# nobodyscool/vkComputeShader_tinyraytracer

Hardware: AMD Instinct MI355X
Metric: Mray/s (primary+secondary) at 1024×768 depth4; 1/2/4/8-GPU scaling (higher is better)
Workload: dtype f32; 1 GPU; C2: 1024x768, 4 spheres + floor + 7616x3808 seeded envmap, depth 4, 1 spp; width=1024, height=768, max_depth=4, spp=1, parallelism=1 GPU

## Files before the change

vkcomputeshader_tinyraytracer_amd/csrc/sky_spans.cpp:

```cpp
#include "sky_spans.h"

#include <algorithm>
#include <cmath>
#include <initializer_list>

#include "../../include/trt/abi.h"
#include "trt_bands.h"

namespace trt {
namespace {

struct Range {
    double lo = 1e300, hi = -1e300;
    void add(double v) {
        lo = std::min(lo, v);
        hi = std::max(hi, v);
    }
};

struct Ball {
    double qx, qy, qz, R, K, dz;
    double ex[2], ey[2];
    double ylo, yhi;
    double a, inv_a;
// ... 21 lines not shown
            const double disc = b * b - a * c;
            if (disc < 0.0) continue;
            const double s = std::sqrt(disc);
            r.add((-b + s) * inv_a);
            r.add((-b - s) * inv_a);
        }
    }
};

struct Seg2 {
    double x0, y0, x1, y1;
    double inv_dy;
};

struct Group {
    bool full = false;
    int nball = 0, nseg = 0;
    Ball ball[4];
    Seg2 seg[12];
};

constexpr double kHuge = 1e6;

bool finite3(const float* v) { return std::isfinite(v[0]) && std::isfinite(v[1]) && std::isfinite(v[2]); }

void prepare_group(const SpanIn& in, const float* cams, uint32_t n, Group& G) {
    const double dz = (double)in.dz;
    double lo[3] = {1e300, 1e300, 1e300}, hi[3] = {-1e300, -1e300, -1e300};
    for (uint32_t f = 0; f < n; ++f) {
        if (!finite3(cams + 3 * f)) {
            G.full = true;
            return;
        }
        for (int a = 0; a < 3; ++a) {
            lo[a] = std::min(lo[a], (double)cams[3 * f + a]);
            hi[a] = std::max(hi[a], (double)cams[3 * f + a]);
        }
    }
    const double oc[3] = {0.5 * (lo[0] + hi[0]), 0.5 * (lo[1] + hi[1]), 0.5 * (lo[2] + hi[2])};
    double rho = 0.0;
    for (uint32_t f = 0; f < n; ++f) {
        double d2 = 0.0;
        for (int a = 0; a < 3; ++a) d2 += ((double)cams[3 * f + a] - oc[a]) * ((double)cams[3 * f + a] - oc[a]);
        rho = std::max(rho, std::sqrt(d2));
    }
    if (!(rho < kHuge) || !(std::fabs(oc[0]) < kHuge) || !(std::fabs(oc[1]) < kHuge) || !(std::fabs(oc[2]) < kHuge)) {
// ... 62 lines not shown
            if (sg.y1 != sg.y0) sg.inv_dy = 1.0 / (sg.y1 - sg.y0);
            G.seg[G.nseg++] = sg;
        }
    }
}

void seg_extent(const Seg2& s, double dy_lo, double dy_hi, Range& r) {
    if (std::max(s.y0, s.y1) < dy_lo || std::min(s.y0, s.y1) > dy_hi) return;
    double t0 = 0.0, t1 = 1.0;
    if (s.inv_dy != 0.0) {
        double ta = (dy_lo - s.y0) * s.inv_dy, tb = (dy_hi - s.y0) * s.inv_dy;
        if (ta > tb) std::swap(ta, tb);
        t0 = std::max(t0, ta);
        t1 = std::min(t1, tb);
        if (t0 > t1) return;
    }
    r.add(s.x0 + t0 * (s.x1 - s.x0));
    r.add(s.x0 + t1 * (s.x1 - s.x0));
}

}

uint32_t sky_spans(const SpanIn& in, const float* cams, uint32_t nframes, uint32_t group_frames, uint32_t* out,
                   uint32_t* ntr_out, uint32_t* shift_out) {
    *ntr_out = 0;
    *shift_out = 0;
    const bool banded = in.band_rows != 0 && in.band_count > 1;
    if (in.rays_in || nframes == 0 || in.width == 0 || in.height == 0) return 0;
    if (banded && (in.band_rows % 8u != 0 || in.band_index >= in.band_count)) return 0;
    const uint32_t rows = banded ? band_group_rows(in.height, in.band_rows, in.band_count, in.band_index) : in.height;
    const uint32_t ntr = (rows + 7u) / 8u, ntx = (in.width + 7u) / 8u;
    if (ntr == 0 || ntr > kSpanWords) return 0;
    uint32_t shift = 1;
    while ((1u << shift) < group_frames && shift < 16) ++shift;
    if (group_frames == 0) shift = 16;
    auto tables = [&](uint32_t s) { return (nframes + (1u << s) - 1u) >> s; };
    while (tables(shift) > kSpanMaxTables || tables(shift) * ntr > kSpanWords) ++shift;
    const uint32_t T = tables(shift);
    *ntr_out = ntr;
    *shift_out = shift;

    const bool sane = in.dz < 0.0f && in.dz > -1e9f;
    const double W = (double)in.width, H = (double)in.height;
    for (uint32_t g = 0; g < T; ++g) {
        uint32_t* tab = out + (size_t)g * ntr;
        const uint32_t f0 = g << shift, n = std::min(nframes - f0, 1u << shift);
        Group G;
        if (sane) prepare_group(in, cams + 3 * (size_t)f0, n, G);
        else G.full = true;
        for (uint32_t tr = 0; tr < ntr; ++tr) {
            if (G.full) {
                tab[tr] = kSpanFull;
                continue;
            }
            const uint32_t k0 = tr * 8u, k1 = std::min(k0 + 7u, rows - 1u);
            const uint32_t y0 = banded ? band_frame_row(k0, in.band_rows, in.band_count, in.band_index) : k0;
            const uint32_t y1 = y0 + (k1 - k0);
            const double dy_hi = H * 0.5 - (double)y0 + 8.0;
            const double dy_lo = H * 0.5 - (double)(y1 + 1u) - ((in.flags & TRT_FLAG_ROW_QUIRK) ? 1.0 : 0.0) - 8.0;
            Range r;
            for (int i = 0; i < G.nball; ++i) G.ball[i].extent(dy_lo, dy_hi, r);
            for (int i = 0; i < G.nseg; ++i) seg_extent(G.seg[i], dy_lo, dy_hi, r);
            if (!(r.lo <= r.hi)) {
                tab[tr] = (r.lo == 1e300 && r.hi == -1e300) ? 0u : kSpanFull;
                continue;
            }
            const double x0 = std::floor(r.lo + W * 0.5 - 0.5), x1 = std::ceil(r.hi + W * 0.5 - 0.5);
            const double c0 = std::max(0.0, std::floor(x0 / 8.0) - 1.0);
            const double c1 = std::min((double)ntx, std::floor(x1 / 8.0) + 2.0);
            tab[tr] = c0 < c1 ? ((uint32_t)c0 | ((uint32_t)c1 << 16)) : 0u;
        }
    }
    return T;
}

}

extern "C" int trt_diag_sky_spans(uint32_t width, uint32_t height, float fov, uint32_t flags, uint32_t band_rows,
                                  uint32_t band_count, uint32_t band_index, int rays_in, const float* spheres,
                                  const float* cams, uint32_t nframes, uint32_t group_frames, uint32_t* out,
                                  uint32_t out_cap, uint32_t* ntr, uint32_t* shift) {
    if (!spheres || !cams || !out || !ntr || !shift) return -1;
    trt::SpanIn in{};
    in.width = width;
    in.height = height;
    in.dz = (float)(-1.0 * ((double)height / (2.0 * std::tan((double)fov / 2.0))));
    in.flags = flags;
    in.band_rows = band_rows;
    in.band_count = band_count;
    in.band_index = band_index;
    in.rays_in = rays_in != 0;
    for (int i = 0; i < 4; ++i)
        for (int a = 0; a < 4; ++a) in.sph[i][a] = spheres[4 * i + a];
    uint32_t tmp[trt::kSpanWords];
    const uint32_t T = trt::sky_spans(in, cams, nframes, group_frames, tmp, ntr, shift);
    if ((size_t)T * *ntr > out_cap) return -1;
    std::copy(tmp, tmp + (size_t)T * *ntr, out);
    return (int)T;
}
```

vkcomputeshader_tinyraytracer_amd/csrc/sky_spans.h:

```cpp
#pragma once

#include <stdint.h>

namespace trt {

constexpr uint32_t kSpanWords = 384;
constexpr uint32_t kSpanMaxTables = 4;
constexpr uint32_t kSpanFull = 0xffff0000u;

struct SpanIn {
    uint32_t width, height;
    float dz;
    uint32_t flags;
    uint32_t band_rows, band_count, band_index;
    bool rays_in;
    float sph[4][4];
};

uint32_t sky_spans(const SpanIn& in, const float* cams, uint32_t nframes, uint32_t group_frames, uint32_t* out,
                   uint32_t* ntr, uint32_t* shift);

}
```

vkcomputeshader_tinyraytracer_amd/csrc/trt_ctx.h:

```cpp
#pragma once

#include <hip/hip_runtime.h>

#include <string>
#include <vector>

#include "../../include/trt/abi.h"
#include "shadow_mask.h"
#include "trt_device.h"

#ifndef TRT_BUILD_MAX_IN_FLIGHT
#define TRT_BUILD_MAX_IN_FLIGHT TRT_MAX_FRAMES_IN_FLIGHT
#endif
static_assert(TRT_BUILD_MAX_IN_FLIGHT >= 1u && TRT_BUILD_MAX_IN_FLIGHT <= TRT_MAX_FRAMES_IN_FLIGHT,
              "TRT_BUILD_MAX_IN_FLIGHT must lie in [1, TRT_MAX_FRAMES_IN_FLIGHT]");

struct trt_ctx {
    int device = 0;
    hipStream_t own_stream = nullptr;
    hipStream_t stream = nullptr;
    std::string err;
    trt_ubo ubo{};
    bool have_scene = false;

    trt::BatchRec* d_batches = nullptr;
    float4* d_nodes = nullptr;
    trt::BvhNode* d_bvh = nullptr;
    trt::Bvh4Node* d_bvh4 = nullptr;
    trt::Bvh4QNode* d_bvh4q = nullptr;
    trt::TriGeo* d_bvh_tris = nullptr;
    uint32_t node_off[11] = {0};
    uint32_t top = 0;
    trt::TriGeo* d_geo = nullptr;
    trt::TriShade* d_shade = nullptr;
    trt::Mat* d_mats = nullptr;
    uint32_t* d_env = nullptr;
    uint2* d_envp = nullptr;
    size_t envp_cap = 0;
    bool envp_ok = false;
    uint32_t nbatch = 0, ntri = 0, nmat = 0, env_w = 0, env_h = 0;
    uint32_t* d_sky = nullptr;
    size_t sky_cap = 0;
    bool sky_on = true, sky_ok = false;
    bool span_on = true;
    uint32_t span_frames = 16;
    uint16_t* d_smask = nullptr;
    bool smask_on = true, smask_ok = false;
    float smask_cell = trt::kShadowCellDefault;
    trt::ShadowMaskIn smask_key{};
    uint32_t smask_nx = 1, smask_nz = 1, smask_rows[2] = {0x0FFF0FFFu, 0x0FFF0FFFu};
    float smask_inv = 0.0f;
    bool smask_fallback = true;
    uint64_t env_gen = 0;
    struct SkyKey {
        uint32_t width, height, flags;
        float dz;
        uint64_t env_gen;
    } sky_key{};

    void* d_out8 = nullptr;
    size_t cap8 = 0;
    void* d_out32 = nullptr;
    size_t cap32 = 0;
    void* d_rays = nullptr;
    size_t caprays = 0;
    unsigned long long* d_counters = nullptr;
    uint32_t num_cus = 256;
    hipEvent_t ev0 = nullptr, ev1 = nullptr;
// ... 80 lines not shown
```

vkcomputeshader_tinyraytracer_amd/csrc/trt_device.h:

```cpp
#pragma once

#include <stdint.h>

#include <hip/hip_runtime.h>

#include "sky_spans.h"

namespace trt {

struct alignas(32) BatchRec {
    float bmin[3];
    float bmax[3];
    int32_t start;
    int32_t count_ni;
};
static_assert(sizeof(BatchRec) == 32, "BatchRec is one s_load_dwordx8");

struct alignas(16) TriGeo {
    float v0[3];
    float e1[3];
    float e2[3];
    float pad[3];
};
static_assert(sizeof(TriGeo) == 48, "TriGeo is 3 x dwordx4");
// ... 151 lines not shown
    float4* __restrict__ diag;
    uint32_t defer;
    uint32_t ev_cap;
    uint32_t shq_cap;
    float4* __restrict__ ev;
    float4* __restrict__ shq;
    uint2* __restrict__ px_ev;
    uint32_t* __restrict__ fb;
    DeferCtr* __restrict__ dctr;
    uint32_t defer_sub;
    uint32_t dframes;
    uint32_t defer_inter;
    uint32_t px_fstride;
    size_t ev_fstride, shq_fstride;
    uint32_t spp_lanes;
    FrameRec fr[kMaxLaunchFrames];
    const uint32_t* __restrict__ sky;
    uint32_t span_tables, span_shift, span_ntr;
    uint32_t span[kSpanWords];
    const uint16_t* __restrict__ smask;
    uint32_t smask_nx, smask_nz;
    float smask_inv;
    uint32_t smask_rows[2];
};
static_assert(sizeof(KArgs) <= 4096, "KArgs fits the 4 KB kernel-argument limit");

}
```

vkcomputeshader_tinyraytracer_amd/csrc/trt_kernel.hip:

```cpp
#include <hip/hip_runtime.h>

#include <algorithm>


#include "../../include/trt/abi.h"
#include "trt_bands.h"
#include "trt_device.h"
#include "trt_math.h"

namespace trt {

__device__ __forceinline__ void wave_lds_sync() { __syncthreads(); }
__device__ __forceinline__ uint32_t lane_id() { return threadIdx.x; }
__device__ __forceinline__ uint32_t lane_rank(uint64_t mask) {
    return __builtin_amdgcn_mbcnt_hi((uint32_t)(mask >> 32), __builtin_amdgcn_mbcnt_lo((uint32_t)mask, 0u));
}

#define TRT_EPS 0.0001f
#ifndef TRT_SKIP_DARK
#define TRT_SKIP_DARK 1
#endif
#ifndef TRT_SPEC_SKIP
#define TRT_SPEC_SKIP 1
#endif
// ... 1878 lines not shown
    }
    if (F.out8) F.out8[o] = pack_rgba8(A, g);
}

__device__ __forceinline__ uint32_t span_word(const KArgs& A, uint32_t tile, uint32_t f) {
    if (A.span_tables == 0u || tile >= A.ntiles) return kSpanFull;
    return A.span[(f >> A.span_shift) * A.span_ntr + tile / A.ntx];
}
__device__ __forceinline__ bool span_outside(const KArgs& A, uint32_t tile, uint32_t span) {
    const uint32_t col = tile % A.ntx;
    return col < (span & 0xffffu) || col >= (span >> 16);
}

__device__ __forceinline__ void sky_tile_store(const KArgs& A, uint32_t tile, const FrameRec& F0, const FrameRec* F1) {
    const uint32_t lane = lane_id();
    const uint32_t x = (tile % A.ntx) * 8u + (lane & 7u), k = (tile / A.ntx) * 8u + (lane >> 3);
    if (x >= A.width || k >= A.rows) return;
    const uint32_t word = A.sky[(size_t)band_row(A, k) * A.width + x];
    const size_t o = (size_t)k * A.width + x;
    if (F0.out8) F0.out8[out_index(A, F0, o)] = word;
    if (F1 && F1->out8) F1->out8[out_index(A, *F1, o)] = word;
}

template <int CAP, bool COUNT, int GEOM, bool SPLIT, bool DEFER = false, bool HYB = SPLIT, bool SKY = false,
          bool SMASK = false>
__device__ __forceinline__ void trace_tile(const KArgs& A, const FrameRec& F, uint32_t tile, Cnt& cnt, float* lds,
                                           float4* slab, uint32_t sub = 0, uint32_t frame = 0) {
    const uint32_t lane = lane_id();
    if (tile >= A.ntiles) return;
    const uint32_t x = (tile % A.ntx) * 8u + (lane & 7u);
    uint32_t k = (tile / A.ntx) * 8u + (lane >> 3);
    const f3 orig = mk(F.cam[0], F.cam[1], F.cam[2]);
    if constexpr (DEFER) {
        const uint32_t S = (!SPLIT && A.defer_sub > 1u) ? A.defer_sub : 1u, rows = 8u / S;
        k = (tile / A.ntx) * 8u + sub * rows + (lane >> 3);
        const bool valid = x < A.width && k < A.rows && (lane >> 3) < rows;
        EvLog L;
        L.S = dscratch(A, frame);
        L.stripe = ((tile * S + sub) * 0x9E3779B1u) >> (32 - 7);
        static_assert(kDeferStripes == 128u, "stripe hash yields 7 bits");
        const size_t o = valid ? (size_t)k * A.width + x : 0u;
        const Seg root = valid ? Seg{orig, primary_dir(A, x, band_row(A, k), 0), 1.0f, 0} : Seg{orig, orig, 0.0f, 0};
        defer_walk<GEOM, SPLIT>(A, lds, slab, L, valid, root, kEvRoot, (uint32_t)o);
        return;
    }
    if (x >= A.width || k >= A.rows) return;
// ... 156 lines not shown
}

template <int GEOM>
constexpr int slab_float4s() {
    return GEOM == 1 ? 64 * 3 : GEOM >= 2 ? (bvh_lds_entries<GEOM>() > 0 ? bvh_lds_entries<GEOM>() * 16 : 1) : 1;
}
#ifndef TRT_G0_WAVES
#define TRT_G0_WAVES 5
#endif
template <int GEOM, int CAP = 99>
constexpr int waves_per_simd() {
    return GEOM == 3 ? (CAP <= 3 ? TRT_G3_WAVES_SHALLOW : TRT_G3_WAVES) : GEOM == 0 ? TRT_G0_WAVES : TRT_WAVES;
}

#ifndef TRT_DEFER_WAVES
#define TRT_DEFER_WAVES 4
#endif
template <int GEOM, int CAP, bool SPLIT, bool DEFER>
constexpr int trace_waves() {
    return (DEFER && GEOM == 3) ? TRT_DEFER_WAVES : waves_per_simd<GEOM, ((SPLIT || DEFER) ? 99 : CAP)>();
}

template <int CAP, bool COUNT, int GEOM, bool SPLIT, bool DEFER, bool HYB, bool SKY, bool SPANS = false,
          bool SMASK = false>
__device__ __forceinline__ void trace_body(const KArgs& A) {
    static_assert(!SPANS || SKY, "the sky spans cull into the sky table");
    static_assert(!SMASK || SPANS, "the occluder masks ride on the span kernel");
    __shared__ float lds[DEFER ? defer_pool_floats() : lds_stack_floats<CAP, GEOM, HYB>()];
    __shared__ float4 slab[slab_float4s<GEOM>()];
    const uint32_t vb = blockIdx.x;
    Cnt cnt;
#ifdef TRT_DIAG_WAVE_CLOCK
    const uint64_t t_start = __builtin_amdgcn_s_memrealtime();
#endif
    uint32_t f = 0, t = vb, tile;
    if (!SPLIT && !DEFER && A.spp_lanes) {
        const uint32_t per = A.ntiles * A.spp;
        f = vb / per;
        const uint32_t r = vb - f * per;
        trace_samples<CAP, COUNT, GEOM>(A, A.fr[f], xcd_tile(A, r / A.spp), r % A.spp, cnt, lds, slab);
        if (COUNT) flush_counts(A, cnt);
        return;
    }
    if (!SPLIT && !DEFER && A.nframes > 1u) {
        if (A.xcd_inter && A.frame_group > 1u && (GEOM == 0 || TRT_MESH_PAIRS)) {
            uint32_t pr;
            tile = inter_tile(A, vb, pr, (A.nframes + 1u) / 2u);
            f = 2u * pr;
#ifndef TRT_DIAG_TRIVIAL
            if constexpr (SPANS) {
                if (span_outside(A, tile, span_word(A, tile, f))) {
                    sky_tile_store(A, tile, A.fr[f], f + 1u < A.nframes ? &A.fr[f + 1u] : nullptr);
                    return;
                }
            }
#endif
            trace_tile<CAP, COUNT, GEOM, SPLIT, DEFER, HYB, SKY, SMASK>(A, A.fr[f], tile, cnt, lds, slab);
            if (f + 1u < A.nframes) trace_tile<CAP, COUNT, GEOM, SPLIT, DEFER, HYB, SKY, SMASK>(A, A.fr[f + 1u], tile, cnt, lds, slab);
            if (COUNT) flush_counts(A, cnt);
            return;
        } else if (A.xcd_inter) {
            tile = inter_tile(A, vb, f, A.nframes);
        } else {
            f = vb / A.ntiles;
            t = vb - f * A.ntiles;
            tile = xcd_tile(A, t, f);
        }
    } else if (DEFER && !SPLIT) {
        const uint32_t Sd = A.defer_sub > 1u ? A.defer_sub : 1u, per = A.ntiles * Sd;
        if (A.defer_inter && A.dframes > 1u) {
            const uint32_t F = A.dframes, per8 = per & ~7u;
            if (vb < F * per8) {
                const uint32_t x = vb & 7u, j = vb >> 3;
// ... 7 lines not shown
        } else {
            f = vb / per;
            t = vb - f * per;
        }
        tile = xcd_tile(A, t / Sd);
        trace_tile<CAP, COUNT, GEOM, SPLIT, DEFER, HYB>(A, A.fr[f], tile, cnt, lds, slab, t % Sd, f);
#ifdef TRT_DIAG_WAVE_CLOCK
        if (threadIdx.x == 0 && A.out32 && A.dframes <= 1u) {
            const uint64_t t_end = __builtin_amdgcn_s_memrealtime();
            uint32_t* rec = reinterpret_cast<uint32_t*>(A.out32) + 4 * (size_t)blockIdx.x;
            uint32_t xcc;
            asm volatile("s_getreg_b32 %0, hwreg(HW_REG_XCC_ID)" : "=s"(xcc));
            rec[0] = tile | ((xcc & 15u) << 28);
            rec[1] = (uint32_t)t_start;
            rec[2] = (uint32_t)(t_end - t_start);
            rec[3] = (uint32_t)(t_start >> 32);
        }
#endif
        return;
    } else {
        tile = xcd_tile(A, t);
    }
#if !defined(TRT_DIAG_TRIVIAL) && !defined(TRT_DIAG_WAVE_CLOCK)
    if constexpr (SPANS) {
        if (span_outside(A, tile, span_word(A, tile, f))) {
            sky_tile_store(A, tile, A.fr[f], nullptr);
            return;
        }
    }
#endif
    trace_tile<CAP, COUNT, GEOM, SPLIT, DEFER, HYB, SKY, SMASK>(A, A.fr[f], tile, cnt, lds, slab);
#ifdef TRT_DIAG_WAVE_CLOCK
    __syncthreads();
    float* clk = A.out32 ? A.out32 : reinterpret_cast<float*>(A.diag);
    if (threadIdx.x == 0 && clk) {
        const uint64_t t_end = __builtin_amdgcn_s_memrealtime();
        uint32_t* rec = reinterpret_cast<uint32_t*>(clk) + 4 * (size_t)blockIdx.x;
        uint32_t xcc;
        asm volatile("s_getreg_b32 %0, hwreg(HW_REG_XCC_ID)" : "=s"(xcc));
        rec[0] = (A.out32 ? xcd_tile(A, blockIdx.x) : (tile | (f << 20))) | ((xcc & 15u) << 28);
        rec[1] = (uint32_t)t_start;
        rec[2] = (uint32_t)(t_end - t_start);
        rec[3] = (uint32_t)(t_start >> 32);
    }
#endif
    if (COUNT) flush_counts(A, cnt);
}

template <int CAP, bool COUNT, int GEOM, bool SPLIT, bool DEFER = false, bool HYB = SPLIT>
__global__ __launch_bounds__(64, (trace_waves<GEOM, CAP, SPLIT, DEFER>())) void trace_kernel(KArgs A) {
    trace_body<CAP, COUNT, GEOM, SPLIT, DEFER, HYB, false>(A);
}

template <int CAP>
__global__ __launch_bounds__(64, (trace_waves<0, CAP, false, false>())) void sky_trace_kernel(KArgs A) {
    trace_body<CAP, false, 0, false, false, false, true, true>(A);
}
template <int CAP>
__global__ __launch_bounds__(64, (trace_waves<0, CAP, false, false>())) void sky_trace_kernel_nospan(KArgs A) {
    trace_body<CAP, false, 0, false, false, false, true, false>(A);
}
template <int CAP>
__global__ __launch_bounds__(64, (trace_waves<0, CAP, false, false>())) void sky_trace_kernel_smask(KArgs A) {
    trace_body<CAP, false, 0, false, false, false, true, true, true>(A);
}

template <int CAP, bool COUNT, int GEOM, bool DEFER = false>
__global__ __launch_bounds__(64, waves_per_simd<GEOM>()) void trace_tasks(KArgs A) {
    __shared__ float lds[DEFER ? defer_pool_floats() : lds_stack_floats<CAP, GEOM, true>()];
    __shared__ float4 slab[slab_float4s<GEOM>()];
    Cnt cnt;
    const uint32_t n = min(*A.q_in_n, A.q_cap);
    for (uint32_t base = blockIdx.x * 64u; base < n; base += gridDim.x * 64u) {
        const uint32_t t = base + threadIdx.x;
        if constexpr (DEFER) {
            const bool valid = t < n;
            Seg root{mk(0.0f, 0.0f, 0.0f), mk(0.0f, 0.0f, 0.0f), 0.0f, 0};
            uint32_t pixel = 0, link = kEvRoot;
            if (valid) {
                const float4* q = reinterpret_cast<const float4*>(A.q_in + t);
                const float4 a = q[0], b = q[1];
                const uint32_t pd = __float_as_uint(b.w);
                pixel = pd >> kTaskDepthBits;
                root = Seg{mk(a.x, a.y, a.z), mk(a.w, b.x, b.y), b.z, (int)(pd & ((1u << kTaskDepthBits) - 1u))};
                link = A.q_link_in[t];
            }
            EvLog L;
// ... 285 lines not shown
        else if (geom == 1) TRT_SPLIT_G(CAP, 1);  \
        else if (geom == 2) TRT_SPLIT_G(CAP, 2);  \
        else TRT_SPLIT_G(CAP, 3);                 \
    } while (0)
        switch (A.split_w) {
        case 2: TRT_SPLIT(1); break;
        case 3: TRT_SPLIT(2); break;
        case 4: TRT_SPLIT(3); break;
        default: TRT_SPLIT(4); break;
        }
#undef TRT_SPLIT
#undef TRT_SPLIT_G
        return hipGetLastError();
    }
    const uint32_t fblocks = A.spp_lanes ? std::max(A.nframes, 1u) * A.spp
                             : A.nframes > 1u && A.xcd_inter && A.frame_group > 1u && (geom == 0 || TRT_MESH_PAIRS)
                                 ? (A.nframes + 1u) / 2u
                                 : std::max(A.nframes, 1u);
    const dim3 fgrid(A.ntiles * fblocks);
    const bool sky = A.sky && geom == 0 && !count && A.spp <= 1 && !A.rays_in && !A.out32;
#define TRT_LAUNCH_G(CAP, G)                                                                             \
    do {                                                                                                 \
        if (count) hipLaunchKernelGGL((trace_kernel<CAP, true, G, false>), fgrid, block, 0, stream, A);  \
        else if (G == 0 && sky && A.span_tables && A.smask) hipLaunchKernelGGL((sky_trace_kernel_smask<CAP>), fgrid, block, 0, stream, A); \
        else if (G == 0 && sky && A.span_tables) hipLaunchKernelGGL((sky_trace_kernel<CAP>), fgrid, block, 0, stream, A); \
        else if (G == 0 && sky) hipLaunchKernelGGL((sky_trace_kernel_nospan<CAP>), fgrid, block, 0, stream, A); \
        else hipLaunchKernelGGL((trace_kernel<CAP, false, G, false>), fgrid, block, 0, stream, A);       \
    } while (0)
#define TRT_LAUNCH(CAP)                          \
    do {                                         \
        if (geom == 0) TRT_LAUNCH_G(CAP, 0);     \
        else if (geom == 1) TRT_LAUNCH_G(CAP, 1); \
        else if (geom == 2) TRT_LAUNCH_G(CAP, 2); \
        else TRT_LAUNCH_G(CAP, 3);               \
    } while (0)
    if (D <= 1) TRT_LAUNCH(0);
    else if (D <= 2) TRT_LAUNCH(1);
    else if (D <= 3) TRT_LAUNCH(2);
    else if (D <= 4) TRT_LAUNCH(3);
    else if (D <= 5) TRT_LAUNCH(4);
    else if (D <= 8) TRT_LAUNCH(7);
    else TRT_LAUNCH(19);
#undef TRT_LAUNCH
#undef TRT_LAUNCH_G
    return hipGetLastError();
}
// ... 83 lines not shown
```

vkcomputeshader_tinyraytracer_amd/csrc/trt_runtime.cpp:

```cpp
#include <hip/hip_runtime.h>

#include <algorithm>
#include <cmath>
#include <cstddef>
#include <cstdio>
#include <cstdlib>
#include <limits>
#include <cstring>
#include <map>
#include <new>
#include <string>
#include <vector>

#include "../../include/trt/abi.h"
#include "jpeg.h"
#include "trt_bands.h"
#include "trt_ctx.h"
#include "trt_device.h"

namespace trt {
hipError_t touch_stream(hipStream_t s, void* scratch) {
    hipError_t e = hipMemsetAsync(scratch, 0, 4, s);
    return e == hipSuccess ? hipStreamSynchronize(s) : e;
}
// ... 179 lines not shown
    }
    if (const char* e = std::getenv("TRT_BVH_WAVES4")) c->bvh_waves4 = std::atoi(e) != 0 ? 1 : 0;
    if (const char* e = std::getenv("TRT_SPP_LANES")) c->spp_lanes = std::atoi(e) != 0;
    if (const char* e = std::getenv("TRT_DEFER_PPW")) {
        const int ppw = std::atoi(e);
        c->defer_sub = ppw == 8 ? 8u : ppw == 16 ? 4u : ppw == 32 ? 2u : ppw == 64 ? 1u : 0u;
    }
    if (const char* e = std::getenv("GPU_MAX_HW_QUEUES")) c->hw_queues = (uint32_t)std::max(1, std::atoi(e));
    if (const char* e = std::getenv("TRT_DEFER_INTER")) c->defer_inter = (uint32_t)std::min(2, std::max(0, std::atoi(e)));
    if (const char* e = std::getenv("TRT_DEFER_GROUP"))
        c->defer_group = (uint32_t)std::min((int)trt::kMaxLaunchFrames, std::max(1, std::atoi(e)));
    if (const char* e = std::getenv("TRT_DEFER_IN_FLIGHT")) {
        c->defer_in_flight = (uint32_t)std::min((int)TRT_BUILD_MAX_IN_FLIGHT, std::max(1, std::atoi(e)));
        c->defer_in_flight_set = true;
    }
    if (const char* e = std::getenv("TRT_XCD_ROT")) c->xcd_rot = (uint32_t)std::min(8, std::max(0, std::atoi(e)));
    if (const char* e = std::getenv("TRT_XCD_SKEW")) c->xcd_skew = (uint32_t)std::min(7, std::max(0, std::atoi(e)));
    if (const char* e = std::getenv("TRT_XCD_INTER")) c->xcd_inter = (uint32_t)std::min(2, std::max(0, std::atoi(e)));
    if (const char* e = std::getenv("TRT_FRAME_GROUP")) c->frame_group = std::min(2, std::max(1, std::atoi(e)));
    if (const char* e = std::getenv("TRT_SKY_TABLE")) c->sky_on = std::atoi(e) != 0;
    if (const char* e = std::getenv("TRT_SKY_SPANS")) c->span_on = std::atoi(e) != 0;
    if (const char* e = std::getenv("TRT_SKY_SPAN_FRAMES")) c->span_frames = (uint32_t)std::min(64, std::max(0, std::atoi(e)));
    if (const char* e = std::getenv("TRT_SHADOW_MASK")) c->smask_on = std::atoi(e) != 0;
    if (const char* e = std::getenv("TRT_SHADOW_MASK_CELL")) {
        const float v = (float)std::atof(e);
        if (v > 0.0f) c->smask_cell = v;
    }
    *out = c;
    return TRT_OK;
}

int trt_destroy(trt_ctx* c) {
    if (!c) return TRT_ERR_INVALID;
    (void)hipSetDevice(c->device);
    if (c->own_stream) (void)hipStreamSynchronize(c->own_stream);
    if (c->stream && c->stream != c->own_stream) (void)hipStreamSynchronize(c->stream);
    (void)hipDeviceSynchronize();
    free_scene(c);
    (void)hipFree(c->d_envp);
    (void)hipFree(c->d_sky);
    (void)hipFree(c->d_smask);
    (void)hipFree(c->d_out8);
    (void)hipFree(c->d_out32);
    (void)hipFree(c->d_rays);
    (void)hipFree(c->d_counters);
    for (hipEvent_t e : c->fev) (void)hipEventDestroy(e);
// ... 321 lines not shown
            (void)hipFree(c->d_sky);
            c->d_sky = nullptr;
            c->sky_cap = 0;
            const hipError_t e = hipMalloc((void**)&c->d_sky, bytes);
            if (e == hipErrorOutOfMemory) {
                (void)hipGetLastError();
                c->d_sky = nullptr;
                c->sky_key = key;
                c->sky_ok = true;
                return TRT_OK;
            }
            HIP_TRY(c, e);
            c->sky_cap = bytes;
        }
        HIP_TRY(c, trt::launch_sky(A, c->d_sky, stream));
        HIP_TRY(c, hipStreamSynchronize(stream));
        c->sky_key = key;
        c->sky_ok = true;
    }
    A.sky = c->d_sky;
    return TRT_OK;
}

void fill_spans(const trt_ctx* c, KArgs& A) {
    A.span_tables = 0;
    if (!A.sky || !c->span_on || A.out32 || A.spp > 1) return;
    trt::SpanIn in{};
    in.width = A.width;
    in.height = A.height;
    in.dz = A.dz;
    in.flags = A.flags;
    in.band_rows = A.band_rows;
    in.band_count = A.band_count;
    in.band_index = A.band_index;
    in.rays_in = A.rays_in != nullptr;
    for (int i = 0; i < 4; ++i) {
        for (int a = 0; a < 3; ++a) in.sph[i][a] = A.sph[i].c[a];
        in.sph[i][3] = A.sph[i].r;
    }
    float cams[3 * trt::kMaxLaunchFrames];
    const uint32_t n = std::min(A.nframes, trt::kMaxLaunchFrames);
    for (uint32_t f = 0; f < n; ++f)
        for (int a = 0; a < 3; ++a) cams[3 * f + a] = A.fr[f].cam[a];
    uint32_t ntr = 0, shift = 0;
    const uint32_t T = trt::sky_spans(in, cams, n, c->span_frames, A.span, &ntr, &shift);
    if (T == 0 || A.ntx == 0 || ntr != A.ntiles / A.ntx) return;
    A.span_tables = T;
    A.span_shift = shift;
    A.span_ntr = ntr;
}

int attach_smask(trt_ctx* c, KArgs& A, hipStream_t stream) {
    A.smask = nullptr;
    if (!A.sky || !A.span_tables || !c->smask_on) return TRT_OK;
    trt::ShadowMaskIn key{};
    for (int j = 0; j < 4; ++j) {
        for (int a = 0; a < 3; ++a) key.sph[j][a] = A.sph[j].c[a];
        key.sph[j][3] = A.sph[j].r;
    }
    std::memcpy(key.light, A.light, sizeof(key.light));
    key.flags = A.flags & TRT_FLAG_SPHERES;
    if (!c->smask_ok || std::memcmp(&key, &c->smask_key, sizeof(key)) != 0) {
        c->smask_ok = false;
        trt::ShadowMask m;
        trt::shadow_mask(key, c->smask_cell, true, m);
        constexpr size_t kCells = 200u * 250u;
        if (m.cells.size() > kCells) trt::shadow_mask(key, c->smask_cell, false, m);
        if (!m.fallback) {
// ... 13 lines not shown
                HIP_TRY(c, hipStreamSynchronize(stream));
            }
        }
        c->smask_nx = m.nx;
        c->smask_nz = m.nz;
        c->smask_inv = m.inv_cell;
        c->smask_rows[0] = m.rows[0] | (m.rows[1] << 16);
        c->smask_rows[1] = m.rows[2] | (m.rows[3] << 16);
        c->smask_fallback = m.fallback;
        c->smask_key = key;
        c->smask_ok = true;
    }
    if (!c->d_smask || c->smask_fallback) return TRT_OK;
    for (uint32_t f = 0; f < A.nframes && f < trt::kMaxLaunchFrames; ++f)
        for (int a = 0; a < 3; ++a)
            if (!(std::fabs(A.fr[f].cam[a]) <= trt::kShadowCamMax)) return TRT_OK;
    A.smask = c->d_smask;
    A.smask_nx = c->smask_nx;
    A.smask_nz = c->smask_nz;
    A.smask_inv = c->smask_inv;
    A.smask_rows[0] = c->smask_rows[0];
    A.smask_rows[1] = c->smask_rows[1];
    return TRT_OK;
}

int check_params(trt_ctx* c, const trt_params* p) {
    if (!p) return fail(c, TRT_ERR_INVALID, "trt_render: null params");
    if (!c->have_scene) return fail(c, TRT_ERR_NOSCENE, "trt_render: no scene uploaded");
    if (p->width == 0 || p->height == 0 || p->width > 65536 || p->height > 65536)
        return fail(c, TRT_ERR_INVALID, "trt_render: image size out of range");
    if (p->max_depth < 1 || p->max_depth > TRT_MAX_DEPTH_LIMIT)
        return fail(c, TRT_ERR_INVALID, "trt_render: max_depth must be 1..20");
    if (p->spp > 4096) return fail(c, TRT_ERR_INVALID, "trt_render: spp must be <= 4096");
    if (p->band_rows && p->band_count > 1 && p->band_index >= p->band_count)
        return fail(c, TRT_ERR_INVALID, "trt_render: band_index >= band_count");
    if ((p->flags & TRT_FLAG_BAND_IN_PLACE) && !(p->flags & TRT_FLAG_DEVICE_PTRS))
        return fail(c, TRT_ERR_INVALID, "trt_render: TRT_FLAG_BAND_IN_PLACE needs TRT_FLAG_DEVICE_PTRS");
    if ((p->flags & TRT_FLAG_ENVMAP) && !c->d_env)
        return fail(c, TRT_ERR_INVALID, "trt_render: TRT_FLAG_ENVMAP without an uploaded envmap");
    return TRT_OK;
}

void fill_args(trt_ctx* c, const trt_params* p, KArgs& A) {
    std::memset(&A, 0, sizeof(A));
    A.width = p->width;
    A.height = p->height;
// ... 342 lines not shown
        HIP_TRY(c, hipStreamCreateWithFlags(&s, hipStreamNonBlocking));
        HIP_TRY(c, trt::touch_stream(s, c->d_counters));
        c->aux.push_back(s);
        hipEvent_t e;
        HIP_TRY(c, hipEventCreateWithFlags(&e, hipEventDisableTiming));
        c->aux_ev.push_back(e);
    }
    if (nfl > 1) {
        if (!c->fork_ev) HIP_TRY(c, hipEventCreateWithFlags(&c->fork_ev, hipEventDisableTiming));
        HIP_TRY(c, hipEventRecord(c->fork_ev, c->stream));
        for (uint32_t k = 0; k + 1 < nfl; ++k) {
            HIP_TRY(c, hipStreamWaitEvent(c->aux[k], c->fork_ev, 0));
            sv.push_back(c->aux[k]);
        }
    }
    for (uint32_t j = 0; j < nl; ++j) {
        const uint32_t i0 = first[j], n = first[j + 1] - i0;
        c->ubo = ubo_of(i0);
        fill_ubo_args(A, c->ubo);
        A.nframes = n;
        for (uint32_t k = 0; k < n; ++k) fill_frame(A.fr[k], ubo_of(i0 + k), frames[i0 + k].out8, frames[i0 + k].in_place);
        fill_spans(c, A);
        if ((rc = attach_smask(c, A, c->stream)) != TRT_OK) return rc;
        uint32_t slot = j % nfl;
        if ((rc = prepare_split(c, p, A, slot, sv[slot])) != TRT_OK) {
            if (c->frames_in_flight || slot == 0 || rc != TRT_ERR_OOM) return rc;
            (void)hipGetLastError();
            c->err.clear();
            nfl = slot;
            c->cur_in_flight = nfl;
            slot = j % nfl;
            if ((rc = prepare_split(c, p, A, slot, sv[slot])) != TRT_OK) return rc;
        }
        hipStream_t st = sv[slot];
        const bool timed = timing && j % every == 0;
        const size_t k = 2 * (size_t)(j / every);
        if (timed) HIP_TRY(c, hipEventRecord(c->fev[k], st));
        HIP_TRY(c, trt::launch_trace(A, st, false));
        if ((rc = fence_split(c, A, slot, st)) != TRT_OK) return rc;
        if (timed) {
            HIP_TRY(c, hipEventRecord(c->fev[k + 1], st));
            c->fev_nframes.push_back(n);
            c->fev_frames = j / every + 1;
        }
    }
    c->ubo = ubo_of(nframes - 1);
// ... 70 lines not shown
            HIP_TRY(c, hipMemcpyAsync(c->d_rays, p->rays_in, bytes, hipMemcpyHostToDevice, c->stream));
            A.rays_in = reinterpret_cast<const float*>(c->d_rays);
        }
    }
    if (out8) {
        if (dev) {
            A.fr[0].out8 = reinterpret_cast<uint32_t*>(out8);
        } else {
            if ((rc = ensure(c, &c->d_out8, &c->cap8, npx * 4, "alloc rgba8")) != TRT_OK) return rc;
            A.fr[0].out8 = reinterpret_cast<uint32_t*>(c->d_out8);
        }
    }
    if (out32) {
        if (dev) {
            A.out32 = out32;
        } else {
            if ((rc = ensure(c, &c->d_out32, &c->cap32, npx * 16, "alloc rgba32f")) != TRT_OK) return rc;
            A.out32 = reinterpret_cast<float*>(c->d_out32);
        }
    }
    if (npx > 0 && (rc = attach_sky(c, A, count, c->stream)) != TRT_OK) return rc;
    fill_spans(c, A);
    if ((rc = attach_smask(c, A, c->stream)) != TRT_OK) return rc;
    const uint32_t slot = render_slot(c, c->stream);
    c->cur_in_flight = 1u;
    if ((rc = prepare_split(c, p, A, slot, c->stream)) != TRT_OK) return rc;
    if (count) HIP_TRY(c, hipMemsetAsync(c->d_counters, 0, 32 * sizeof(unsigned long long), c->stream));
    if (timing) HIP_TRY(c, hipEventRecord(c->ev0, c->stream));
    if (npx > 0) HIP_TRY(c, trt::launch_trace(A, c->stream, count));
    if ((rc = fence_split(c, A, slot, c->stream)) != TRT_OK) return rc;
    if (timing) HIP_TRY(c, hipEventRecord(c->ev1, c->stream));
    if (out8 && !dev)
        HIP_TRY(c, hipMemcpyAsync(out8, c->d_out8, npx * 4, hipMemcpyDeviceToHost, c->stream));
    if (out32 && !dev)
        HIP_TRY(c, hipMemcpyAsync(out32, c->d_out32, npx * 16, hipMemcpyDeviceToHost, c->stream));
    unsigned long long cnt[32] = {0};
    if (count)
        HIP_TRY(c, hipMemcpyAsync(cnt, c->d_counters, sizeof(cnt), hipMemcpyDeviceToHost, c->stream));
    if (!dev || count || timing) HIP_TRY(c, hipStreamSynchronize(c->stream));
    if (st) {
        st->primary_rays = cnt[0];
        st->secondary_rays = cnt[1];
        st->shadow_rays = cnt[2];
        st->misses = cnt[3];
        st->tri_nearest = cnt[4];
        st->sphere_tests = cnt[5];
// ... 212 lines not shown
```

Measured before the change: 118,200 Mray/s.

## Classify floor-only tiles via sphere spans and shade them with a specialized floor path

Extends the host-side sky span computation to also produce a per-row sphere-only span, packs both spans into one byte-packed word, and adds a kernel variant that sends tiles outside the sphere span but inside the floor span to a lightweight floor-only shader (plane hit, checker, shadow-masked lights) instead of the full trace. This is meant to skip full scene traversal and reflection/refraction work for tiles that can only see the floor or sky. It is enabled only for multi-frame batches (nframes > 1) with spans and a shadow mask, so single-frame renders keep the old path. It adds host packing work, a new kernel instantiation, and a correctness risk if the conservative sphere bounds miss reflections or refractions.

```diff
diff --git a/vkcomputeshader_tinyraytracer_amd/csrc/sky_spans.cpp b/vkcomputeshader_tinyraytracer_amd/csrc/sky_spans.cpp
--- a/vkcomputeshader_tinyraytracer_amd/csrc/sky_spans.cpp
+++ b/vkcomputeshader_tinyraytracer_amd/csrc/sky_spans.cpp
@@ -67,6 +67,17 @@
 
 constexpr double kHuge = 1e6;
 
+inline double floor_d(double x) {
+    if (!(std::fabs(x) < 4e15)) return std::floor(x);
+    const double t = (double)(int64_t)x;
+    return t > x ? t - 1.0 : t;
+}
+inline double ceil_d(double x) {
+    if (!(std::fabs(x) < 4e15)) return std::ceil(x);
+    const double t = (double)(int64_t)x;
+    return t < x ? t + 1.0 : t;
+}
+
 bool finite3(const float* v) { return std::isfinite(v[0]) && std::isfinite(v[1]) && std::isfinite(v[2]); }
 
 void prepare_group(const SpanIn& in, const float* cams, uint32_t n, Group& G) {
@@ -175,7 +186,7 @@
 }
 
 uint32_t sky_spans(const SpanIn& in, const float* cams, uint32_t nframes, uint32_t group_frames, uint32_t* out,
-                   uint32_t* ntr_out, uint32_t* shift_out) {
+                   uint32_t* ntr_out, uint32_t* shift_out, uint32_t* sph_out) {
     *ntr_out = 0;
     *shift_out = 0;
     const bool banded = in.band_rows != 0 && in.band_count > 1;
@@ -197,6 +208,7 @@
     const double W = (double)in.width, H = (double)in.height;
     for (uint32_t g = 0; g < T; ++g) {
         uint32_t* tab = out + (size_t)g * ntr;
+        uint32_t* stab = sph_out ? sph_out + (size_t)g * ntr : nullptr;
         const uint32_t f0 = g << shift, n = std::min(nframes - f0, 1u << shift);
         Group G;
         if (sane) prepare_group(in, cams + 3 * (size_t)f0, n, G);
@@ -204,6 +216,7 @@
         for (uint32_t tr = 0; tr < ntr; ++tr) {
             if (G.full) {
                 tab[tr] = kSpanFull;
+                if (stab) stab[tr] = kSpanFull;
                 continue;
             }
             const uint32_t k0 = tr * 8u, k1 = std::min(k0 + 7u, rows - 1u);
@@ -211,17 +224,22 @@
             const uint32_t y1 = y0 + (k1 - k0);
             const double dy_hi = H * 0.5 - (double)y0 + 8.0;
             const double dy_lo = H * 0.5 - (double)(y1 + 1u) - ((in.flags & TRT_FLAG_ROW_QUIRK) ? 1.0 : 0.0) - 8.0;
-            Range r;
-            for (int i = 0; i < G.nball; ++i) G.ball[i].extent(dy_lo, dy_hi, r);
+            Range rb;
+            for (int i = 0; i < G.nball; ++i) G.ball[i].extent(dy_lo, dy_hi, rb);
+            Range r = rb;
             for (int i = 0; i < G.nseg; ++i) seg_extent(G.seg[i], dy_lo, dy_hi, r);
-            if (!(r.lo <= r.hi)) {
-                tab[tr] = (r.lo == 1e300 && r.hi == -1e300) ? 0u : kSpanFull;
-                continue;
-            }
-            const double x0 = std::floor(r.lo + W * 0.5 - 0.5), x1 = std::ceil(r.hi + W * 0.5 - 0.5);
-            const double c0 = std::max(0.0, std::floor(x0 / 8.0) - 1.0);
-            const double c1 = std::min((double)ntx, std::floor(x1 / 8.0) + 2.0);
-            tab[tr] = c0 < c1 ? ((uint32_t)c0 | ((uint32_t)c1 << 16)) : 0u;
+            auto word = [&](const Range& e) -> uint32_t {
+                if (!(e.lo <= e.hi)) return (e.lo == 1e300 && e.hi == -1e300) ? 0u : kSpanFull;
+                const double x0 = floor_d(e.lo + W * 0.5 - 0.5), x1 = ceil_d(e.hi + W * 0.5 - 0.5);
+                const double c0 = std::max(0.0, floor_d(x0 * 0.125) - 1.0);
+                const double c1 = std::min((double)ntx, floor_d(x1 * 0.125) + 2.0);
+                return c0 < c1 ? ((uint32_t)c0 | ((uint32_t)c1 << 16)) : 0u;
+            };
+            tab[tr] = word(r);
+            if (stab) {
+                const uint32_t w = (rb.lo == r.lo && rb.hi == r.hi) ? tab[tr] : word(rb);
+                stab[tr] = (w == kSpanFull && tab[tr] != kSpanFull) ? tab[tr] : w;
+            }
         }
     }
     return T;
@@ -229,10 +247,10 @@
 
 }
 
-extern "C" int trt_diag_sky_spans(uint32_t width, uint32_t height, float fov, uint32_t flags, uint32_t band_rows,
-                                  uint32_t band_count, uint32_t band_index, int rays_in, const float* spheres,
-                                  const float* cams, uint32_t nframes, uint32_t group_frames, uint32_t* out,
-                                  uint32_t out_cap, uint32_t* ntr, uint32_t* shift) {
+static int diag_spans(bool sphere, uint32_t width, uint32_t height, float fov, uint32_t flags, uint32_t band_rows,
+                      uint32_t band_count, uint32_t band_index, int rays_in, const float* spheres, const float* cams,
+                      uint32_t nframes, uint32_t group_frames, uint32_t* out, uint32_t out_cap, uint32_t* ntr,
+                      uint32_t* shift) {
     if (!spheres || !cams || !out || !ntr || !shift) return -1;
     trt::SpanIn in{};
     in.width = width;
@@ -245,9 +263,26 @@
     in.rays_in = rays_in != 0;
     for (int i = 0; i < 4; ++i)
         for (int a = 0; a < 4; ++a) in.sph[i][a] = spheres[4 * i + a];
-    uint32_t tmp[trt::kSpanWords];
-    const uint32_t T = trt::sky_spans(in, cams, nframes, group_frames, tmp, ntr, shift);
+    uint32_t tmp[trt::kSpanWords], stmp[trt::kSpanWords];
+    const uint32_t T = trt::sky_spans(in, cams, nframes, group_frames, tmp, ntr, shift, stmp);
     if ((size_t)T * *ntr > out_cap) return -1;
-    std::copy(tmp, tmp + (size_t)T * *ntr, out);
+    const uint32_t* src = sphere ? stmp : tmp;
+    std::copy(src, src + (size_t)T * *ntr, out);
     return (int)T;
 }
+
+extern "C" int trt_diag_sky_spans(uint32_t width, uint32_t height, float fov, uint32_t flags, uint32_t band_rows,
+                                  uint32_t band_count, uint32_t band_index, int rays_in, const float* spheres,
+                                  const float* cams, uint32_t nframes, uint32_t group_frames, uint32_t* out,
+                                  uint32_t out_cap, uint32_t* ntr, uint32_t* shift) {
+    return diag_spans(false, width, height, fov, flags, band_rows, band_count, band_index, rays_in, spheres, cams, nframes,
+                      group_frames, out, out_cap, ntr, shift);
+}
+
+extern "C" int trt_diag_sphere_spans(uint32_t width, uint32_t height, float fov, uint32_t flags, uint32_t band_rows,
+                                     uint32_t band_count, uint32_t band_index, int rays_in, const float* spheres,
+                                     const float* cams, uint32_t nframes, uint32_t group_frames, uint32_t* out,
+                                     uint32_t out_cap, uint32_t* ntr, uint32_t* shift) {
+    return diag_spans(true, width, height, fov, flags, band_rows, band_count, band_index, rays_in, spheres, cams, nframes,
+                      group_frames, out, out_cap, ntr, shift);
+}
diff --git a/vkcomputeshader_tinyraytracer_amd/csrc/sky_spans.h b/vkcomputeshader_tinyraytracer_amd/csrc/sky_spans.h
--- a/vkcomputeshader_tinyraytracer_amd/csrc/sky_spans.h
+++ b/vkcomputeshader_tinyraytracer_amd/csrc/sky_spans.h
@@ -18,6 +18,13 @@
 };
 
 uint32_t sky_spans(const SpanIn& in, const float* cams, uint32_t nframes, uint32_t group_frames, uint32_t* out,
-                   uint32_t* ntr, uint32_t* shift);
+                   uint32_t* ntr, uint32_t* shift, uint32_t* sph_out = nullptr);
+
+constexpr uint32_t kFloorPackMaxNtx = 255;
+constexpr uint32_t kFloorPackFull = 0xff00ff00u;
+inline uint32_t floor_pack(uint32_t span, uint32_t sph) {
+    auto b = [](uint32_t v) { return v < 255u ? v : 255u; };
+    return b(span & 0xffffu) | b(span >> 16) << 8 | b(sph & 0xffffu) << 16 | b(sph >> 16) << 24;
+}
 
 }
diff --git a/vkcomputeshader_tinyraytracer_amd/csrc/trt_ctx.h b/vkcomputeshader_tinyraytracer_amd/csrc/trt_ctx.h
--- a/vkcomputeshader_tinyraytracer_amd/csrc/trt_ctx.h
+++ b/vkcomputeshader_tinyraytracer_amd/csrc/trt_ctx.h
@@ -44,6 +44,8 @@
     bool sky_on = true, sky_ok = false;
     bool span_on = true;
     uint32_t span_frames = 16;
+    bool floor_on = true;
+    uint32_t sph_span[trt::kSpanWords] = {};
     uint16_t* d_smask = nullptr;
     bool smask_on = true, smask_ok = false;
     float smask_cell = trt::kShadowCellDefault;
diff --git a/vkcomputeshader_tinyraytracer_amd/csrc/trt_device.h b/vkcomputeshader_tinyraytracer_amd/csrc/trt_device.h
--- a/vkcomputeshader_tinyraytracer_amd/csrc/trt_device.h
+++ b/vkcomputeshader_tinyraytracer_amd/csrc/trt_device.h
@@ -197,6 +197,7 @@
     uint32_t smask_nx, smask_nz;
     float smask_inv;
     uint32_t smask_rows[2];
+    uint32_t floor_class;
 };
 static_assert(sizeof(KArgs) <= 4096, "KArgs fits the 4 KB kernel-argument limit");
 
diff --git a/vkcomputeshader_tinyraytracer_amd/csrc/trt_kernel.hip b/vkcomputeshader_tinyraytracer_amd/csrc/trt_kernel.hip
--- a/vkcomputeshader_tinyraytracer_amd/csrc/trt_kernel.hip
+++ b/vkcomputeshader_tinyraytracer_amd/csrc/trt_kernel.hip
@@ -1924,6 +1924,88 @@
     if (F1 && F1->out8) F1->out8[out_index(A, *F1, o)] = word;
 }
 
+__device__ __forceinline__ uint32_t floor_span_word(const KArgs& A, uint32_t tile, uint32_t f) {
+    if (tile >= A.ntiles) return kFloorPackFull;
+    return A.span[(f >> A.span_shift) * A.span_ntr + tile / A.ntx];
+}
+__device__ __forceinline__ bool floor_span_outside(uint32_t col, uint32_t w) {
+    return col < (w & 0xffu) || col >= ((w >> 8) & 0xffu);
+}
+__device__ __forceinline__ bool floor_sphere_outside(uint32_t col, uint32_t w) {
+    return col < ((w >> 16) & 0xffu) || col >= (w >> 24);
+}
+
+__device__ __forceinline__ void floor_frame(const KArgs& A, const FrameRec& F, f3 d, uint32_t word, size_t o, Cnt& cnt,
+                                            float4* slab) {
+    const f3 orig = mk(F.cam[0], F.cam[1], F.cam[2]);
+    float t = 1e10f;
+    bool hit = false;
+    if (A.flags & TRT_FLAG_FLOOR) {
+        if (fabsf(d.y) > TRT_EPS) {
+            const float tf = div_rn(-(orig.y + 4.0f), d.y);
+            if (tf > TRT_EPS && tf < t) {
+                const f3 pf = add(orig, muls(d, tf));
+                if (fabsf(pf.x) < 10.0f && pf.z < -5.0f && pf.z > -30.0f) {
+                    t = tf;
+                    hit = true;
+                }
+            }
+        }
+    }
+    if (!hit) {
+        if (F.out8) F.out8[out_index(A, F, o)] = word;
+        return;
+    }
+    const f3 p = add(orig, muls(d, t));
+    const int ix = min(max((int)((p.x + 10.0f) * A.smask_inv), 0), (int)A.smask_nx - 1);
+    const int iz = min(max((int)((p.z + 30.0f) * A.smask_inv), 0), (int)A.smask_nz - 1);
+    uint32_t sm = A.smask[(uint32_t)iz * A.smask_nx + (uint32_t)ix];
+#ifdef TRT_DIAG_NO_FLOOR_SHADOW
+    sm = 0u;
+#endif
+    const f3 n = mk(0.0f, 1.0f, 0.0f);
+    float c1 = 0.3f, c2 = 0.3f;
+    if (A.flags & TRT_FLAG_CHECKER) {
+        const float m = floorf(p.x * 0.5f + 1024.0f) + floorf(p.z * 0.5f);
+        const float mod2 = m - 2.0f * floorf(m / 2.0f);
+        if (!(mod2 == 0.0f)) {
+            c1 = 0.2f;
+            c2 = 0.1f;
+        }
+    }
+    const float alb0 = 2.0f, alb1 = 0.0f;
+    const f3 kdv = mk(0.3f, c1, c2);
+    f3 diffuse = mk(0.0f, 0.0f, 0.0f);
+    const f3 specular = mk(0.0f, 0.0f, 0.0f);
+#pragma unroll
+    for (int i = 0; i < 3; ++i) {
+        const f3 L = mk(A.light[i][0], A.light[i][1], A.light[i][2]);
+        float dist;
+        const f3 ld = normalize_len3(sub(L, p), dist);
+        const f3 so = dot3(ld, n) < 0.0f ? sub(p, muls(n, TRT_EPS)) : add(p, muls(n, TRT_EPS));
+        const float diff = 1.0f * fmaxf(0.0f, dot3(n, ld));
+        const bool matters = TRT_SKIP_DARK == 0 || diff != 0.0f;
+        if (!matters) continue;
+        if (shadow_intersect<false, 0, true>(A, so, ld, dist, cnt, slab, sm >> (4 * i))) continue;
+        diffuse = add(diffuse, muls(kdv, diff));
+    }
+    const f3 c = add(mk(0.0f, 0.0f, 0.0f), muls(add(muls(diffuse, alb0), muls(specular, alb1)), 1.0f));
+    store_pixel(A, F, o, mk(clamp01(c.x), clamp01(c.y), clamp01(c.z)));
+}
+
+__device__ __forceinline__ void floor_tile(const KArgs& A, uint32_t tile, const FrameRec& F0, const FrameRec* F1, Cnt& cnt,
+                                           float4* slab) {
+    const uint32_t lane = lane_id();
+    const uint32_t x = (tile % A.ntx) * 8u + (lane & 7u), k = (tile / A.ntx) * 8u + (lane >> 3);
+    if (x >= A.width || k >= A.rows) return;
+    const uint32_t y = band_row(A, k);
+    const size_t o = (size_t)k * A.width + x;
+    const f3 d = primary_dir(A, x, y, 0);
+    const uint32_t word = A.sky[(size_t)y * A.width + x];
+    floor_frame(A, F0, d, word, o, cnt, slab);
+    if (F1) floor_frame(A, *F1, d, word, o, cnt, slab);
+}
+
 template <int CAP, bool COUNT, int GEOM, bool SPLIT, bool DEFER = false, bool HYB = SPLIT, bool SKY = false,
           bool SMASK = false>
 __device__ __forceinline__ void trace_tile(const KArgs& A, const FrameRec& F, uint32_t tile, Cnt& cnt, float* lds,
@@ -2126,10 +2208,11 @@
 }
 
 template <int CAP, bool COUNT, int GEOM, bool SPLIT, bool DEFER, bool HYB, bool SKY, bool SPANS = false,
-          bool SMASK = false>
+          bool SMASK = false, bool FLOORC = false>
 __device__ __forceinline__ void trace_body(const KArgs& A) {
     static_assert(!SPANS || SKY, "the sky spans cull into the sky table");
     static_assert(!SMASK || SPANS, "the occluder masks ride on the span kernel");
+    static_assert(!FLOORC || SMASK, "the floor class rides on the mask kernel");
     __shared__ float lds[DEFER ? defer_pool_floats() : lds_stack_floats<CAP, GEOM, HYB>()];
     __shared__ float4 slab[slab_float4s<GEOM>()];
     const uint32_t vb = blockIdx.x;
@@ -2152,7 +2235,22 @@
             tile = inter_tile(A, vb, pr, (A.nframes + 1u) / 2u);
             f = 2u * pr;
 #ifndef TRT_DIAG_TRIVIAL
-            if constexpr (SPANS) {
+            if constexpr (FLOORC) {
+                const uint32_t w = floor_span_word(A, tile, f), col = tile % A.ntx;
+                const FrameRec* F1 = f + 1u < A.nframes ? &A.fr[f + 1u] : nullptr;
+                if (floor_span_outside(col, w)) {
+                    sky_tile_store(A, tile, A.fr[f], F1);
+                    return;
+                }
+                if (floor_sphere_outside(col, w)) {
+#ifdef TRT_DIAG_FLOOR_SKY
+                    sky_tile_store(A, tile, A.fr[f], F1);
+#else
+                    floor_tile(A, tile, A.fr[f], F1, cnt, slab);
+#endif
+                    return;
+                }
+            } else if constexpr (SPANS) {
                 if (span_outside(A, tile, span_word(A, tile, f))) {
                     sky_tile_store(A, tile, A.fr[f], f + 1u < A.nframes ? &A.fr[f + 1u] : nullptr);
                     return;
@@ -2206,7 +2304,21 @@
         tile = xcd_tile(A, t);
     }
 #if !defined(TRT_DIAG_TRIVIAL) && !defined(TRT_DIAG_WAVE_CLOCK)
-    if constexpr (SPANS) {
+    if constexpr (FLOORC) {
+        const uint32_t w = floor_span_word(A, tile, f), col = tile % A.ntx;
+        if (floor_span_outside(col, w)) {
+            sky_tile_store(A, tile, A.fr[f], nullptr);
+            return;
+        }
+        if (floor_sphere_outside(col, w)) {
+#ifdef TRT_DIAG_FLOOR_SKY
+            sky_tile_store(A, tile, A.fr[f], nullptr);
+#else
+            floor_tile(A, tile, A.fr[f], nullptr, cnt, slab);
+#endif
+            return;
+        }
+    } else if constexpr (SPANS) {
         if (span_outside(A, tile, span_word(A, tile, f))) {
             sky_tile_store(A, tile, A.fr[f], nullptr);
             return;
@@ -2247,6 +2359,11 @@
 template <int CAP>
 __global__ __launch_bounds__(64, (trace_waves<0, CAP, false, false>())) void sky_trace_kernel_smask(KArgs A) {
     trace_body<CAP, false, 0, false, false, false, true, true, true>(A);
+}
+
+template <int CAP>
+__global__ __launch_bounds__(64, (trace_waves<0, CAP, false, false>())) void sky_trace_kernel_floor(KArgs A) {
+    trace_body<CAP, false, 0, false, false, false, true, true, true, true>(A);
 }
 
 template <int CAP, bool COUNT, int GEOM, bool DEFER = false>
@@ -2578,6 +2695,7 @@
 #define TRT_LAUNCH_G(CAP, G)                                                                             \
     do {                                                                                                 \
         if (count) hipLaunchKernelGGL((trace_kernel<CAP, true, G, false>), fgrid, block, 0, stream, A);  \
+        else if (G == 0 && sky && A.span_tables && A.smask && A.floor_class) hipLaunchKernelGGL((sky_trace_kernel_floor<CAP>), fgrid, block, 0, stream, A); \
         else if (G == 0 && sky && A.span_tables && A.smask) hipLaunchKernelGGL((sky_trace_kernel_smask<CAP>), fgrid, block, 0, stream, A); \
         else if (G == 0 && sky && A.span_tables) hipLaunchKernelGGL((sky_trace_kernel<CAP>), fgrid, block, 0, stream, A); \
         else if (G == 0 && sky) hipLaunchKernelGGL((sky_trace_kernel_nospan<CAP>), fgrid, block, 0, stream, A); \
diff --git a/vkcomputeshader_tinyraytracer_amd/csrc/trt_runtime.cpp b/vkcomputeshader_tinyraytracer_amd/csrc/trt_runtime.cpp
--- a/vkcomputeshader_tinyraytracer_amd/csrc/trt_runtime.cpp
+++ b/vkcomputeshader_tinyraytracer_amd/csrc/trt_runtime.cpp
@@ -225,6 +225,7 @@
     if (const char* e = std::getenv("TRT_SKY_SPANS")) c->span_on = std::atoi(e) != 0;
     if (const char* e = std::getenv("TRT_SKY_SPAN_FRAMES")) c->span_frames = (uint32_t)std::min(64, std::max(0, std::atoi(e)));
     if (const char* e = std::getenv("TRT_SHADOW_MASK")) c->smask_on = std::atoi(e) != 0;
+    if (const char* e = std::getenv("TRT_FLOOR_CLASS")) c->floor_on = std::atoi(e) != 0;
     if (const char* e = std::getenv("TRT_SHADOW_MASK_CELL")) {
         const float v = (float)std::atof(e);
         if (v > 0.0f) c->smask_cell = v;
@@ -592,8 +593,9 @@
     return TRT_OK;
 }
 
-void fill_spans(const trt_ctx* c, KArgs& A) {
+void fill_spans(trt_ctx* c, KArgs& A) {
     A.span_tables = 0;
+    A.floor_class = 0;
     if (!A.sky || !c->span_on || A.out32 || A.spp > 1) return;
     trt::SpanIn in{};
     in.width = A.width;
@@ -613,7 +615,7 @@
     for (uint32_t f = 0; f < n; ++f)
         for (int a = 0; a < 3; ++a) cams[3 * f + a] = A.fr[f].cam[a];
     uint32_t ntr = 0, shift = 0;
-    const uint32_t T = trt::sky_spans(in, cams, n, c->span_frames, A.span, &ntr, &shift);
+    const uint32_t T = trt::sky_spans(in, cams, n, c->span_frames, A.span, &ntr, &shift, c->floor_on && A.nframes > 1u ? c->sph_span : nullptr);
     if (T == 0 || A.ntx == 0 || ntr != A.ntiles / A.ntx) return;
     A.span_tables = T;
     A.span_shift = shift;
@@ -673,6 +675,15 @@
     A.smask_rows[0] = c->smask_rows[0];
     A.smask_rows[1] = c->smask_rows[1];
     return TRT_OK;
+}
+
+void attach_floor_class(const trt_ctx* c, KArgs& A) {
+    A.floor_class = 0;
+    if (!c->floor_on || A.nframes < 2u || !A.span_tables || !A.smask || A.ntx > trt::kFloorPackMaxNtx) return;
+    if (!(A.flags & TRT_FLAG_FLOOR) || !(A.flags & TRT_FLAG_SPHERES)) return;
+    const uint32_t words = A.span_tables * A.span_ntr;
+    for (uint32_t i = 0; i < words; ++i) A.span[i] = trt::floor_pack(A.span[i], c->sph_span[i]);
+    A.floor_class = 1;
 }
 
 int check_params(trt_ctx* c, const trt_params* p) {
@@ -1061,6 +1072,7 @@
         for (uint32_t k = 0; k < n; ++k) fill_frame(A.fr[k], ubo_of(i0 + k), frames[i0 + k].out8, frames[i0 + k].in_place);
         fill_spans(c, A);
         if ((rc = attach_smask(c, A, c->stream)) != TRT_OK) return rc;
+        attach_floor_class(c, A);
         uint32_t slot = j % nfl;
         if ((rc = prepare_split(c, p, A, slot, sv[slot])) != TRT_OK) {
             if (c->frames_in_flight || slot == 0 || rc != TRT_ERR_OOM) return rc;
@@ -1177,6 +1189,7 @@
     if (npx > 0 && (rc = attach_sky(c, A, count, c->stream)) != TRT_OK) return rc;
     fill_spans(c, A);
     if ((rc = attach_smask(c, A, c->stream)) != TRT_OK) return rc;
+    attach_floor_class(c, A);
     const uint32_t slot = render_slot(c, c->stream);
     c->cur_in_flight = 1u;
     if ((rc = prepare_split(c, p, A, slot, c->stream)) != TRT_OK) return rc;
```

Result: faster. 131,000 Mray/s (median of 6 runs) (+10.8%).
